# ilyakurdyukov/jpeg-quantsmooth

Hardware: AMD Instinct MI355X
Metric: 8x8 blocks/s at q=3 niter=3 (higher is better)
Workload: dtype f32

## Files before the change

### jpeg-quantsmooth_amd/csrc/qs_device.h

```cpp
#pragma once
#include <stdint.h>

#define QS_APRON_X 16
#define QS_LDS_PITCH 65
#define QS_TAB_MAX 272

enum {
  QS_DIAGONALS = 1, QS_JOINT_YUV = 2, QS_UPSAMPLE_UV = 4, QS_LOW_QUALITY = 8,
  QS_NO_REBALANCE = 16, QS_NO_REBALANCE_UV = 32, QS_TRANSCODE = 64
};

struct QsConsts {
  int32_t nat[64];
  int32_t q[64];
  int32_t qraw[64];
  int32_t x1[64];
  int32_t x2[64];
  float   range[64];
  int32_t qn[64], x1n[64], x2n[64];
  int32_t tab_size;
  int32_t pad[15];
  float   tab[64 * QS_TAB_MAX];
  int32_t rec[64][4];
};
enum {
  QS_REC_H_ANY = 1,
  QS_REC_H_SKIP4 = 2,
  QS_REC_H_EVEN = 4,
  QS_REC_V_ANY = 8,
  QS_REC_V_SKIP4 = 16,
  QS_REC_V_EVEN = 32,
  QS_REC_LDS_SHIFT = 6,
  QS_REC_NXT_SHIFT = 12,
  QS_REC_Q1 = 1 << 21
};

static inline int qs_plane_pitch(int wblk) {
  return ((wblk * 8 + QS_APRON_X + 1) + 63) & ~63;
}

#define QS_MAX_PLANES 56
struct QsPlaneRef {
  const QsConsts* cst;
  int16_t* coef;
  uint8_t* plane;
  int32_t* status;
  int32_t wblk, hblk, pitch;
  int32_t mode;
  uint8_t* plane_next;
};
enum {
  QS_PLANE_REBALANCE = 1,
  QS_PLANE_REP_TOP = 2,
  QS_PLANE_REP_BOT = 4
};
struct QsPlaneAux {
  const uint8_t* p[QS_MAX_PLANES];
};
struct QsPlaneSet {
  int32_t n, pad;
  int32_t wave0[QS_MAX_PLANES + 2];
  QsPlaneRef ref[QS_MAX_PLANES];
};
```

### jpeg-quantsmooth_amd/csrc/qs_kernels.hip

```cpp
#include <hip/hip_runtime.h>
#include <stdint.h>
#include <stdlib.h>
#include "qs_device.h"



__device__ __forceinline__ void wave_lds_sync() {
  __builtin_amdgcn_fence(__ATOMIC_RELEASE, "wavefront");
  __builtin_amdgcn_wave_barrier();
  __builtin_amdgcn_fence(__ATOMIC_ACQUIRE, "wavefront");
}

__device__ __forceinline__ uint32_t mulc(uint32_t a, int c) {
  return (uint32_t)__mul24((int)a, c);
}

__device__ __forceinline__ uint32_t lshl13_add(uint32_t x, uint32_t b) {
  uint32_t r;
  asm("v_lshl_add_u32 %0, %1, 13, %2" : "=v"(r) : "v"(x), "v"(b));
  return r;
}

__device__ __forceinline__ void idct8(uint32_t (&v)[8], uint32_t bias) {
  uint32_t z1, z2, z3, z4, z5, t0, t1, t2, t3, e0, e1, e2, e3;
// ... 176 lines not shown
               "ds_read_i16 %6, %16 offset:780\n\tds_read_i16 %7, %16 offset:782\n\t" \
               "ds_read_i16 %8, %16 offset:1040\n\tds_read_i16 %9, %16 offset:1042\n\t" \
               "ds_read_i16 %10, %16 offset:1300\n\tds_read_i16 %11, %16 offset:1302\n\t" \
               "ds_read_i16 %12, %16 offset:1560\n\tds_read_i16 %13, %16 offset:1562\n\t" \
               "ds_read_i16 %14, %16 offset:1820\n\tds_read_i16 %15, %16 offset:1822\n\t" \
               "s_waitcnt lgkmcnt(0)" \
               : "=&v"(W[(N0) + 0]), "=&v"(W[(N0) + 1]), "=&v"(W[(N0) + 2]), "=&v"(W[(N0) + 3]), \
                 "=&v"(W[(N0) + 4]), "=&v"(W[(N0) + 5]), "=&v"(W[(N0) + 6]), "=&v"(W[(N0) + 7]), \
                 "=&v"(W[(N0) + 8]), "=&v"(W[(N0) + 9]), "=&v"(W[(N0) + 10]), "=&v"(W[(N0) + 11]), \
                 "=&v"(W[(N0) + 12]), "=&v"(W[(N0) + 13]), "=&v"(W[(N0) + 14]), "=&v"(W[(N0) + 15]) \
               : "v"(BASE) : "memory")
__device__ __forceinline__ void lds_read_block_i16(const uint32_t* col, uint32_t (&ws)[64]) {
  typedef const __attribute__((address_space(3))) uint32_t* lds_ptr;
  const uint32_t a0 = (uint32_t)(uintptr_t)(lds_ptr)col;
  const uint32_t a1 = a0 + 8 * 260, a2 = a0 + 16 * 260, a3 = a0 + 24 * 260;
  QS_LDS16_GROUP(a0, ws, 0);
  QS_LDS16_GROUP(a1, ws, 16);
  QS_LDS16_GROUP(a2, ws, 32);
  QS_LDS16_GROUP(a3, ws, 48);
}

#define QS_PIX_SCALE 0.000244140625f
#define QS_TERM_D(D, W) { \
    float u_ = __builtin_amdgcn_fmed3f(Rs - __builtin_fabsf(D), 0.0f, 1.0f); \
    float t_ = u_ * u_; \
    float x_ = (D) * t_; \
    float y_ = (W) * t_; \
    num = num + x_ * y_; \
    den = den + y_ * y_; }
#define QS_TERM(A, B, W) { float d_ = (A) - (B); QS_TERM_D(d_, W) }

typedef float qs_w16 __attribute__((ext_vector_type(16)));
typedef int qs_i4 __attribute__((ext_vector_type(4)));
#define QS_SWAIT(BUF) asm volatile("s_waitcnt lgkmcnt(0)" : "+s"(BUF) : : "memory")

#define QS_WAVES_PER_WG 4
#define QS_SMOOTH_MIN_WAVES 3
#define QS_RESIDENT_WG (256 * QS_SMOOTH_MIN_WAVES * 4 / QS_WAVES_PER_WG)
#define QS_PRIO_SLOW 3
#define QS_PRIO_TERMS 0

#define QS_TERM_OPT(COND, A, B, W) { float d_, t_; \
        asm volatile( \
          "s_cmp_lg_u32 %[c], 0\n\t" \
          "s_cbranch_scc1 1f\n\t" \
          "v_sub_f32 %[d], %[a], %[b]\n\t" \
          "v_sub_f32 %[t], %[r], |%[d]| clamp\n\t" \
          "v_mul_f32 %[t], %[t], %[t]\n\t" \
          "v_mul_f32 %[d], %[d], %[t]\n\t" \
          "v_mul_f32 %[t], %[w], %[t]\n\t" \
          "v_mul_f32 %[d], %[d], %[t]\n\t" \
          "v_add_f32 %[n], %[n], %[d]\n\t" \
          "v_mul_f32 %[d], %[t], %[t]\n\t" \
          "v_add_f32 %[e], %[e], %[d]\n" \
          "1:" \
          : [n] "+v"(num), [e] "+v"(den), [d] "=&v"(d_), [t] "=&v"(t_) \
          : [a] "v"(A), [b] "v"(B), [w] "s"(W), [r] "s"(Rs), [c] "s"(COND) : "scc"); }
#define QS_TERM_ASM(A, B, W) { float d_, t_; \
        asm volatile( \
          "v_sub_f32 %[d], %[a], %[b]\n\t" \
          "v_sub_f32 %[t], %[r], |%[d]| clamp\n\t" \
          "v_mul_f32 %[t], %[t], %[t]\n\t" \
          "v_mul_f32 %[d], %[d], %[t]\n\t" \
          "v_mul_f32 %[t], %[w], %[t]\n\t" \
          "v_mul_f32 %[d], %[d], %[t]\n\t" \
          "v_add_f32 %[n], %[n], %[d]\n\t" \
          "v_mul_f32 %[d], %[t], %[t]\n\t" \
          "v_add_f32 %[e], %[e], %[d]" \
          : [n] "+v"(num), [e] "+v"(den), [d] "=&v"(d_), [t] "=&v"(t_) \
          : [a] "v"(A), [b] "v"(B), [w] "s"(W), [r] "s"(Rs)); }

#define QS_TERM_D_ASM(D, W) { float d_, t_; \
        asm volatile( \
          "v_sub_f32 %[t], %[r], |%[a]| clamp\n\t" \
          "v_mul_f32 %[t], %[t], %[t]\n\t" \
          "v_mul_f32 %[d], %[a], %[t]\n\t" \
          "v_mul_f32 %[t], %[w], %[t]\n\t" \
          "v_mul_f32 %[d], %[d], %[t]\n\t" \
          "v_add_f32 %[n], %[n], %[d]\n\t" \
          "v_mul_f32 %[d], %[t], %[t]\n\t" \
          "v_add_f32 %[e], %[e], %[d]" \
          : [n] "+v"(num), [e] "+v"(den), [d] "=&v"(d_), [t] "=&v"(t_) \
          : [a] "v"(D), [w] "s"(W), [r] "s"(Rs)); }
#define QS_HOIST 20
#ifndef QS_HOIST_DIAG
#define QS_HOIST_DIAG 32
#endif
#ifndef QS_Q1_SKIP
#define QS_Q1_SKIP 1
#endif
#ifndef QS_STASH
#define QS_STASH 1
#endif

#define QS_SMOOTH_KERNEL_NAME qs_smooth_plane_kernel
#include "qs_smooth_kernel.inc"
#undef QS_SMOOTH_KERNEL_NAME
#define QS_SMOOTH_KERNEL_NAME qs_smooth_set_kernel
#define QS_SMOOTH_SET 1
#include "qs_smooth_kernel.inc"
#undef QS_SMOOTH_KERNEL_NAME
#undef QS_SMOOTH_SET

#define QS_DP_KERNEL_NAME qs_smooth_dp_kernel
#include "qs_smooth_dp_kernel.inc"
#undef QS_DP_KERNEL_NAME
#define QS_DP_KERNEL_NAME qs_smooth_dp_set_kernel
#define QS_DP_SET 1
#include "qs_smooth_dp_kernel.inc"
#undef QS_DP_KERNEL_NAME
#undef QS_DP_SET

__global__ void __launch_bounds__(256)
qs_clamp_kernel(int16_t* __restrict__ coef, size_t nvec) {
  size_t i = (size_t)blockIdx.x * 256 + threadIdx.x;
  const size_t stride = (size_t)gridDim.x * 256;
  uint4* p = reinterpret_cast<uint4*>(coef);
  for (; i < nvec; i += stride) {
    uint4 v = p[i];
    uint32_t d[4] = {v.x, v.y, v.z, v.w};
#pragma unroll
    for (int c = 0; c < 4; ++c) {
      int lo = (int16_t)(d[c] & 0xffff), hi = (int32_t)d[c] >> 16;
      lo = min(max(lo, -1023), 1023); hi = min(max(hi, -1023), 1023);
      d[c] = ((uint32_t)lo & 0xffffu) | ((uint32_t)hi << 16);
    }
    p[i] = make_uint4(d[0], d[1], d[2], d[3]);
  }
}

__global__ void __launch_bounds__(256)
qs_dequant_kernel(const QsConsts* __restrict__ cst, int16_t* __restrict__ coef, size_t nvec) {
  size_t i = (size_t)blockIdx.x * 256 + threadIdx.x;
  const size_t stride = (size_t)gridDim.x * 256;
  uint4* p = reinterpret_cast<uint4*>(coef);
  for (; i < nvec; i += stride) {
    uint4 v = p[i];
    uint32_t d[4] = {v.x, v.y, v.z, v.w};
    const int j = (int)(i & 7);
#pragma unroll
    for (int c = 0; c < 4; ++c) {
      int lo = (int16_t)(d[c] & 0xffff), hi = (int32_t)d[c] >> 16;
      lo *= cst->qraw[j * 8 + c * 2]; hi *= cst->qraw[j * 8 + c * 2 + 1];
      d[c] = ((uint32_t)lo & 0xffffu) | ((uint32_t)hi << 16);
    }
    p[i] = make_uint4(d[0], d[1], d[2], d[3]);
  }
}

#include "qs_launch.h"

void qs_launch_idct_plane(const QsConsts* cst, int16_t* coef, uint8_t* plane, int wblk, int hblk,
                          int first, int rep_top, int rep_bot, int* status, hipStream_t s) {
  const int nblk = wblk * hblk;
  hipLaunchKernelGGL(qs_idct_plane_kernel, dim3((nblk + 255) / 256), dim3(256), 0, s,
                     cst, coef, plane, wblk, hblk, qs_plane_pitch(wblk), first, rep_top, rep_bot, status);
}

#define QS_DP_WAVES 4
static int qs_dp_waves(int groups) {
  static const int on = [] { const char* v = getenv("QS_HIP_DP"); return v ? atoi(v) : 1; }();
  static const int lim = [] { const char* v = getenv("QS_HIP_DP_GROUPS"); return v ? atoi(v) : 768; }();
  static const int lim2 = [] { const char* v = getenv("QS_HIP_DP_GROUPS2"); return v ? atoi(v) : 1536; }();
  if (!on) return 0;
  return groups <= lim ? QS_DP_WAVES : groups <= lim2 ? 2 : 0;
}

void qs_launch_smooth_plane(const QsConsts* cst, int16_t* coef, const uint8_t* plane, uint8_t* plane_next, int rep_top, int rep_bot,
                            int wblk, int hblk, int diag, int rebalance, int final_clamp, int blk_begin, int blk_end, hipStream_t s) {
// ... 53 lines not shown
```

### jpeg-quantsmooth_amd/csrc/qs_smooth_kernel.inc

```
template <bool DIAG>
__global__ void __launch_bounds__(64 * QS_WAVES_PER_WG, QS_SMOOTH_MIN_WAVES)
#ifdef QS_SMOOTH_SET
QS_SMOOTH_KERNEL_NAME(const QsPlaneSet set, int final_clamp) {
  __shared__ uint32_t lds_all[QS_WAVES_PER_WG][32 * QS_LDS_PITCH];
#if QS_STASH
  __shared__ uint32_t stash_all[QS_WAVES_PER_WG][2 * 8 * 64];
#endif
  const int lane = threadIdx.x & 63, wave = threadIdx.x >> 6;
  uint32_t* lds = lds_all[wave];
  uint32_t* col = lds + lane;
  const int gw = __builtin_amdgcn_readfirstlane((int)(blockIdx.x * QS_WAVES_PER_WG + wave));
  if (gw >= set.wave0[set.n]) return;
  const int pi = qs_set_find(set, gw);
  const QsConsts* __restrict__ cst = set.ref[pi].cst;
  int16_t* __restrict__ coef = set.ref[pi].coef;
  const uint8_t* __restrict__ plane = set.ref[pi].plane;
  const int wblk = set.ref[pi].wblk, hblk = set.ref[pi].hblk, pitch = set.ref[pi].pitch;
  const int rebalance = set.ref[pi].mode & QS_PLANE_REBALANCE;
  const int nblk = wblk * hblk;
  const int base = (gw - set.wave0[pi]) * 64;
  (void)hblk;
#else
QS_SMOOTH_KERNEL_NAME(const QsConsts* __restrict__ cst, int16_t* __restrict__ coef,
                       const uint8_t* __restrict__ plane, uint8_t* __restrict__ plane_next, int rep,
                       int wblk, int hblk, int pitch,
                       int rebalance, int final_clamp, int blk_begin, int blk_end) {
  __shared__ uint32_t lds_all[QS_WAVES_PER_WG][32 * QS_LDS_PITCH];
#if QS_STASH
  __shared__ uint32_t stash_all[QS_WAVES_PER_WG][2 * 8 * 64];
#endif
  const int lane = threadIdx.x & 63, wave = threadIdx.x >> 6;
  uint32_t* lds = lds_all[wave];
  uint32_t* col = lds + lane;
  const int nblk = blk_end;
  const int base = blk_begin + (blockIdx.x * QS_WAVES_PER_WG + wave) * 64;
#endif
  if (base >= nblk) return;
  const int tail_prio = __builtin_amdgcn_readfirstlane(
      (gridDim.x > QS_RESIDENT_WG && blockIdx.x >= (gridDim.x / QS_RESIDENT_WG) * QS_RESIDENT_WG) ? 1 : 0);
  const int nvec = min(64, nblk - base) * 8;
#ifdef QS_STAGGER
  { unsigned hwid; asm volatile("s_getreg_b32 %0, hwreg(HW_REG_HW_ID)" : "=s"(hwid)); if (hwid & 1u) __builtin_amdgcn_s_sleep(QS_STAGGER); }
#endif

  uint4* gsrc = reinterpret_cast<uint4*>(coef) + (size_t)base * 8;
  {
    const int m0 = (lane & 7) * 4;
#pragma unroll
    for (int j = 0; j < 8; ++j) {
      const int idx = j * 64 + lane;
      uint4 v = make_uint4(0, 0, 0, 0);
      if (idx < nvec) v = gsrc[idx];
      uint32_t* dst = lds + m0 * QS_LDS_PITCH + (j * 8 + (lane >> 3));
      dst[0] = v.x; dst[QS_LDS_PITCH] = v.y; dst[2 * QS_LDS_PITCH] = v.z; dst[3 * QS_LDS_PITCH] = v.w;
    }
  }

  const int blk = min(base + lane, nblk - 1);
  const int by = blk / wblk, bx = blk - by * wblk;
  const uint8_t* org = plane + (size_t)(by * 8 + 1) * pitch + QS_APRON_X + bx * 8;
  uint32_t edge[8];
  {
    const uint2 t = *reinterpret_cast<const uint2*>(org - pitch);
    const uint2 b = *reinterpret_cast<const uint2*>(org + (size_t)8 * pitch);
    edge[0] = t.x; edge[1] = t.y; edge[2] = b.x; edge[3] = b.y;
    uint32_t l[8], r[8];
#pragma unroll
    for (int y = 0; y < 8; ++y) {
      l[y] = org[(ptrdiff_t)y * pitch - 1];
      r[y] = org[(ptrdiff_t)y * pitch + 8];
    }
    edge[4] = l[0] | (l[1] << 8) | (l[2] << 16) | (l[3] << 24);
    edge[5] = l[4] | (l[5] << 8) | (l[6] << 16) | (l[7] << 24);
    edge[6] = r[0] | (r[1] << 8) | (r[2] << 16) | (r[3] << 24);
    edge[7] = r[4] | (r[5] << 8) | (r[6] << 16) | (r[7] << 24);
  }
  wave_lds_sync();

  constexpr int TS = DIAG ? 272 : 160;
  float px[64];
  float bd[32];
  constexpr int NH = DIAG ? QS_HOIST_DIAG : QS_HOIST;
  float hd[NH];

  int kfirst = 63;
#if QS_STASH
  int stash_hi = 0;
#endif
  uint32_t chg = 0;
  long long reb_m0 = 0, reb_m1 = 0;
  const float* tabp = cst->tab;
  const int32_t* recp = &cst->rec[0][0];
  qs_w16 WA, WB;
  qs_i4 REC;
  qs_i4 RECN;
  asm volatile("s_load_dwordx4 %0, %2, %3\n\ts_load_dwordx16 %1, %4, %5\n\ts_waitcnt lgkmcnt(0)"
               : "=&s"(REC), "=&s"(WA) : "s"(recp), "s"(63u * 16u), "s"(tabp), "s"((uint32_t)63 * (TS * 4)) : "memory");
  RECN = REC;

#pragma unroll 1
  for (int g = 0; g < 14; ++g) {
    __builtin_amdgcn_s_setprio(QS_PRIO_SLOW);
    if (g == 0 || __builtin_amdgcn_ballot_w64(chg != 0) != 0) {
      chg = 0;
      uint32_t ws[64];
      lds_read_block_i16(col, ws);
#if QS_STASH
      {
        uint32_t* stash = stash_all[wave] + lane;
#pragma unroll
        for (int x = 0; x < 8; ++x) {
          uint32_t c[8];
          const bool low = x <= 1, high = x >= 6;
          const int slot = (x == 0 || x == 7) ? 0 : 1;
          bool reuse = false, store = false;
          if (low) { reuse = g >= 1 && g <= 7 - x; store = g == 0; }
          if (high) {
            const int fin = 15 - x;
            const bool have = (stash_hi >> (x - 6)) & 1;
            reuse = g >= fin && have; store = g >= fin && !have;
          }
          if ((low || high) && reuse) {
#pragma unroll
            for (int j = 0; j < 8; ++j) c[j] = stash[(slot * 8 + j) * 64];
          } else {
#pragma unroll
            for (int j = 0; j < 8; ++j) c[j] = ws[j * 8 + x];
            idct8(c, 1024u);
#pragma unroll
            for (int j = 0; j < 8; ++j) c[j] = (uint32_t)((int32_t)c[j] >> 11);
            if ((low || high) && store) {
#pragma unroll
              for (int j = 0; j < 8; ++j) stash[(slot * 8 + j) * 64] = c[j];
              if (high) stash_hi |= 1 << (x - 6);
            }
          }
#pragma unroll
          for (int j = 0; j < 8; ++j) ws[j * 8 + x] = c[j];
        }
      }
#else
      idct_pass1(ws);
#endif
#pragma unroll
      for (int y = 0; y < 8; ++y) {
        uint32_t row[8]; float o[8];
#pragma unroll
        for (int j = 0; j < 8; ++j) row[j] = ws[y * 8 + j];
        idct_pass2_row_f(row, o);
#pragma unroll
        for (int j = 0; j < 8; ++j) px[y * 8 + j] = o[j];
      }
#pragma unroll
      for (int e = 0; e < 8; ++e) asm volatile("" : "+v"(edge[e]));
#pragma unroll
      for (int x = 0; x < 8; ++x) {
        bd[x]      = px[x]         - pix_from_byte(edge[0 + (x >> 2)], x & 3);
        bd[8 + x]  = px[56 + x]    - pix_from_byte(edge[2 + (x >> 2)], x & 3);
        bd[16 + x] = px[x * 8]     - pix_from_byte(edge[4 + (x >> 2)], x & 3);
        bd[24 + x] = px[x * 8 + 7] - pix_from_byte(edge[6 + (x >> 2)], x & 3);
      }
#pragma unroll
      for (int t = 0; t < NH; ++t) hd[t] = px[(t / 7) * 8 + t % 7] - px[(t / 7) * 8 + t % 7 + 1];
    }
    const int len = min(g + 1, 15 - g);
    const int klast = max(kfirst - len + 1, 1);
#pragma unroll 1
    for (int k = kfirst; k >= klast; --k) {
#pragma unroll
      for (int p = 0; p < 64; ++p) asm volatile("" : "+v"(px[p]));
      const int md = REC[3];
      const int x2k = (REC[0] >> 16) & 31, qk = REC[1] & 0xffff, x1k = REC[1] >> 16;
      const uint32_t lds_off = ((uint32_t)md >> QS_REC_LDS_SHIFT) & 0x3fffu;
      int rs_bits = REC[2];
      asm volatile("" : "+s"(rs_bits));
      const float Rs = __builtin_bit_cast(float, rs_bits);
      const uint32_t kb = (uint32_t)k * (TS * 4);
      const uint32_t kb_nxt = kb - (uint32_t)(TS * 4);
      const uint32_t kb_s = (uint32_t)__builtin_amdgcn_readfirstlane((int)kb);
      const uint32_t kb_nxt_s = (uint32_t)__builtin_amdgcn_readfirstlane((int)kb_nxt);
      const uint32_t next_first = kb_nxt + (((uint32_t)md >> QS_REC_NXT_SHIFT) & 0x100u);
      const uint32_t after_V = DIAG ? kb + 640u : next_first;
      const uint32_t after_B = (md & QS_REC_V_ANY) ? kb + 384u : after_V;
#if QS_Q1_SKIP
      if (__builtin_expect(md & QS_REC_Q1, 0)) {
        {
          const int c0 = *reinterpret_cast<lds_i16*>(reinterpret_cast<char*>(col) + lds_off);
          reb_m0 += (long long)(c0 * c0);
          reb_m1 += (long long)(c0 * c0);
        }
        asm volatile("s_load_dwordx16 %0, %2, %3\n\ts_load_dwordx4 %1, %4, %5\n\ts_waitcnt lgkmcnt(0)"
                     : "=&s"(WA), "=&s"(RECN)
                     : "s"(tabp), "s"((uint32_t)__builtin_amdgcn_readfirstlane((int)next_first)), "s"(recp),
                       "s"((uint32_t)(k - 1) * 16u) : "memory");
        REC = RECN;
      } else
#endif
      {
      float num = 0.0f, den = 0.0f;
      asm volatile("s_setprio %c1\n\ts_cmp_eq_u32 %0, 0\n\ts_cbranch_scc1 1f\n\ts_setprio %c2\n1:"
                   : : "s"(tail_prio), "i"(QS_PRIO_TERMS), "i"(QS_PRIO_TERMS + 1) : "scc");

#define QS_ROW_D(W, Y) { \
        _Pragma("unroll") for (int x = 0; x < 7; ++x) { \
          QS_TERM(px[(Y) * 8 + x], px[(Y) * 8 + x + 9], W[x]) \
          QS_TERM(px[(Y) * 8 + x + 1], px[(Y) * 8 + x + 8], W[8 + x]) } }
#define QS_EDGE16(W, J0) { \
        _Pragma("unroll") for (int j = 0; j < 16; ++j) QS_TERM_D(bd[(J0) + j], W[j]) }
#define QS_HOISTED_TERM(T, WT) else if ((T) < NH) QS_TERM_D_ASM(hd[(T) % NH], WT)
#define QS_ROWS_H_M(W, Y0, MODE) { \
        _Pragma("unroll") for (int yy = 0; yy < 2; ++yy) \
        _Pragma("unroll") for (int x = 0; x < 7; ++x) { \
          if (((MODE) == 2 && (x & 1)) || ((MODE) == 1 && x == 3)) {} \
          QS_HOISTED_TERM(((Y0) + yy) * 7 + x, W[yy * 8 + x]) \
          else QS_TERM_ASM(px[((Y0) + yy) * 8 + x], px[((Y0) + yy) * 8 + x + 1], W[yy * 8 + x]) } }
#define QS_ROWS_V_M(W, Y0, NY, MODE) { \
        _Pragma("unroll") for (int yy = 0; yy < (NY); ++yy) \
        _Pragma("unroll") for (int x = 0; x < 8; ++x) { \
          if (((MODE) == 2 && (((Y0) + yy) & 1)) || ((MODE) == 1 && (Y0) + yy == 3)) {} \
          else QS_TERM_ASM(px[((Y0) + yy) * 8 + x], px[((Y0) + yy) * 8 + x + 8], W[yy * 8 + x]) } }

      const uint32_t rec_next = (uint32_t)(k - 1) * 16u;
#define QS_ISSUE(NXT, BYTEOFF) \
      asm volatile("s_load_dwordx16 %0, %3, %4" : "=&s"(NXT), "+v"(num), "+v"(den) \
                   : "s"(tabp), "s"((uint32_t)__builtin_amdgcn_readfirstlane((int)(BYTEOFF))) : "memory")
#define QS_ISSUE_K(NXT, IMM) \
      asm volatile("s_load_dwordx16 %0, %3, %4 offset:%c5" : "=&s"(NXT), "+v"(num), "+v"(den) \
                   : "s"(tabp), "s"(kb_s), "i"(IMM) : "memory")
#define QS_LAND(NXT) asm volatile("s_waitcnt lgkmcnt(0)" : "+s"(NXT), "+v"(num), "+v"(den) : : "memory")
#define QS_ISSUE_R(NXT, BYTEOFF) \
      asm volatile("s_load_dwordx16 %0, %4, %5\n\ts_load_dwordx4 %1, %6, %7" : "=&s"(NXT), "=&s"(RECN), "+v"(num), "+v"(den) \
                   : "s"(tabp), "s"((uint32_t)__builtin_amdgcn_readfirstlane((int)(BYTEOFF))), "s"(recp), "s"(rec_next) : "memory")
#define QS_LAND_R(NXT) asm volatile("s_waitcnt lgkmcnt(0)" : "+s"(NXT), "+s"(RECN), "+v"(num), "+v"(den) : : "memory")
#define QS_T4(O) "s_load_dword %1, %4, %5 offset:" #O "\n\ts_load_dword %1, %4, %5 offset:" #O "+0x40\n\ts_load_dword %1, %4, %5 offset:" #O "+0x80\n\ts_load_dword %1, %4, %5 offset:" #O "+0xc0\n\t"
#define QS_ISSUE_T(NXT, IMM) \
      uint32_t touch; \
      if (DIAG) asm volatile("s_load_dwordx16 %0, %4, %6 offset:%c7\n\t" QS_T4(0x0) QS_T4(0x100) QS_T4(0x200) QS_T4(0x300) "s_load_dword %1, %4, %5 offset:0x400" \
                   : "=&s"(NXT), "=&s"(touch), "+v"(num), "+v"(den) \
                   : "s"(tabp), "s"(kb_nxt_s), "s"(kb_s), "i"(IMM) : "memory"); \
      else      asm volatile("s_load_dwordx16 %0, %4, %6 offset:%c7\n\t" QS_T4(0x0) QS_T4(0x100) "s_load_dword %1, %4, %5 offset:0x200\n\ts_load_dword %1, %4, %5 offset:0x240" \
                   : "=&s"(NXT), "=&s"(touch), "+v"(num), "+v"(den) \
                   : "s"(tabp), "s"(kb_nxt_s), "s"(kb_s), "i"(IMM) : "memory")
#define QS_LAND_T(NXT) asm volatile("s_waitcnt lgkmcnt(0)" : "+s"(NXT), "+s"(touch), "+v"(num), "+v"(den) : : "memory")
#define QS_H_SECTION(MODE) { \
        QS_ISSUE_K(WB, 64);  QS_ROWS_H_M(WA, 0, MODE) QS_LAND(WB); \
        QS_ISSUE_K(WA, 128); QS_ROWS_H_M(WB, 2, MODE) QS_LAND(WA); \
        QS_ISSUE_K(WB, 192); QS_ROWS_H_M(WA, 4, MODE) QS_LAND(WB); \
        QS_ISSUE_K(WA, 256); QS_ROWS_H_M(WB, 6, MODE) QS_LAND(WA); }
      if (md & QS_REC_H_ANY) {
        if (md & QS_REC_H_SKIP4) QS_H_SECTION(2)
        else if (md & QS_REC_H_EVEN) QS_H_SECTION(1)
        else QS_H_SECTION(0)
      }
      QS_ISSUE_T(WB, 320); QS_EDGE16(WA, 0) QS_LAND_T(WB);
      if (!DIAG && !(md & QS_REC_V_ANY)) { QS_ISSUE_R(WA, after_B); QS_EDGE16(WB, 16) QS_LAND_R(WA); }
      else                   { QS_ISSUE(WA, after_B);   QS_EDGE16(WB, 16) QS_LAND(WA); }
#define QS_V_SECTION(MODE) { \
        QS_ISSUE_K(WB, 448); QS_ROWS_V_M(WA, 0, 2, MODE) QS_LAND(WB); \
        QS_ISSUE_K(WA, 512); QS_ROWS_V_M(WB, 2, 2, MODE) QS_LAND(WA); \
        QS_ISSUE_K(WB, 576); QS_ROWS_V_M(WA, 4, 2, MODE) QS_LAND(WB); \
        if (!DIAG) { QS_ISSUE_R(WA, after_V); QS_ROWS_V_M(WB, 6, 1, MODE) QS_LAND_R(WA); } \
        else       { QS_ISSUE(WA, after_V);   QS_ROWS_V_M(WB, 6, 1, MODE) QS_LAND(WA); } }
      if (md & QS_REC_V_ANY) {
        if (md & QS_REC_V_SKIP4) QS_V_SECTION(2)
        else if (md & QS_REC_V_EVEN) QS_V_SECTION(1)
        else QS_V_SECTION(0)
      }
      if (DIAG) {
        QS_ISSUE_K(WB, 704);  QS_ROW_D(WA, 0) QS_LAND(WB);
        QS_ISSUE_K(WA, 768);  QS_ROW_D(WB, 1) QS_LAND(WA);
        QS_ISSUE_K(WB, 832);  QS_ROW_D(WA, 2) QS_LAND(WB);
        QS_ISSUE_K(WA, 896);  QS_ROW_D(WB, 3) QS_LAND(WA);
        QS_ISSUE_K(WB, 960);  QS_ROW_D(WA, 4) QS_LAND(WB);
        QS_ISSUE_K(WA, 1024); QS_ROW_D(WB, 5) QS_LAND(WA);
        QS_ISSUE_R(WB, next_first); QS_ROW_D(WA, 6) QS_LAND_R(WB);
        WA = WB;
      }
#undef QS_ROWS_H_M
#undef QS_HOISTED_TERM
#undef QS_ROWS_V_M
#undef QS_H_SECTION
#undef QS_V_SECTION
#undef QS_ISSUE
#undef QS_ISSUE_K
#undef QS_LAND
#undef QS_ISSUE_R
#undef QS_LAND_R
#undef QS_ISSUE_T
#undef QS_LAND_T
#undef QS_T4

      __builtin_amdgcn_s_setprio(QS_PRIO_SLOW);
      lds_i16* const cptr = reinterpret_cast<lds_i16*>(reinterpret_cast<char*>(col) + lds_off);
      const int c0 = *cptr;
      const int r = f2i_x86(round_half_away((num / den) * 4096.0f));
      {
        int orig, lo, hi;
        interval(c0, qk, x1k, x2k, orig, lo, hi);
        int v = (int)((uint32_t)c0 - (uint32_t)r);
        v = min(max(v, lo), hi);
        *cptr = (lds_i16)v;
        chg |= (uint32_t)(v ^ c0);
        if (rebalance) {
          reb_m0 += (long long)(v * orig);
          reb_m1 += (long long)(orig * orig);
        }
      }
      REC = RECN;
      }
    }
    kfirst = klast - 1;
  }
  QS_SWAIT(WA);

  if (rebalance) {
    const long long m0 = reb_m0, m1 = reb_m1;
    if (m1 > m0) {
      const int mul = (int)(((m1 << 13) + (m0 >> 1)) / m0);
#pragma unroll 9
      for (int n = 1; n < 64; ++n) {
        const int c = lds_coef(col, n);
        int orig, lo, hi;
        interval(c, cst->qn[n], cst->x1n[n], cst->x2n[n], orig, lo, hi);
        int v = (c * mul + 0x1000) >> 13;
        v = min(max(v, lo), hi);
        lds_set_coef(col, n, v);
      }
    }
  }
  wave_lds_sync();

  {
    int lane2 = lane;
    asm volatile("" : "+v"(lane2));
    const int lane = lane2;
    const int m0 = (lane & 7) * 4;
#pragma unroll
    for (int j = 0; j < 8; ++j) {
      const int idx = j * 64 + lane;
      const uint32_t* s = lds + m0 * QS_LDS_PITCH + (j * 8 + (lane >> 3));
      uint32_t d[4] = {s[0], s[QS_LDS_PITCH], s[2 * QS_LDS_PITCH], s[3 * QS_LDS_PITCH]};
      if (final_clamp) {
#pragma unroll
        for (int c = 0; c < 4; ++c) {
          int lo = (int16_t)(d[c] & 0xffff), hi = (int32_t)d[c] >> 16;
          lo = min(max(lo, -1023), 1023); hi = min(max(hi, -1023), 1023);
          d[c] = ((uint32_t)lo & 0xffffu) | ((uint32_t)hi << 16);
        }
      }
      if (idx < nvec) gsrc[idx] = make_uint4(d[0], d[1], d[2], d[3]);
    }
  }

#ifdef QS_SMOOTH_SET
  int pi2 = pi;
  asm volatile("" : "+s"(pi2));
  uint8_t* __restrict__ plane_next = set.ref[pi2].plane_next;
  const int rep = set.ref[pi2].mode, wblk2 = set.ref[pi2].wblk, hblk2 = set.ref[pi2].hblk, pitch2 = set.ref[pi2].pitch;
#else
  const int wblk2 = wblk, hblk2 = hblk, pitch2 = pitch;
#endif
  if (plane_next) {
    uint32_t ws[64];
    lds_read_block_i16(col, ws);
    if (base + lane < nblk)
      idct_ws_to_plane(ws, plane_next, wblk2, hblk2, pitch2, rep & QS_PLANE_REP_TOP, rep & QS_PLANE_REP_BOT, base + lane);
  }
}

#undef QS_ROW_D
#undef QS_EDGE16
```

### jpeg-quantsmooth_amd/csrc/qs_tables.cpp

```cpp
#include <stdarg.h>
#include <math.h>
#include <mutex>

#include "qs_xfer.h"

static thread_local char g_err[512] = "";

int qs_fail(int code, const char* fmt, ...) {
  va_list ap; va_start(ap, fmt);
  vsnprintf(g_err, sizeof(g_err), fmt, ap);
  va_end(ap);
  return code;
}


extern "C" const char* qs_hip_last_error(void) { return g_err; }

extern "C" int qs_hip_device_count(void) {
  int n = 0;
  if (hipGetDeviceCount(&n) != hipSuccess) { (void)hipGetLastError(); return 0; }
  return n;
}

extern "C" size_t qs_hip_consts_bytes(void) { return sizeof(QsConsts); }
extern "C" size_t qs_hip_plane_pitch(int wblk) { return (size_t)qs_plane_pitch(wblk); }
extern "C" size_t qs_hip_plane_bytes(int wblk, int hblk) {
  return (size_t)qs_plane_pitch(wblk) * ((size_t)hblk * 8 + 2) + 64;
}
extern "C" size_t qs_hip_plane_row_offset(int wblk, int y) {
  return (size_t)qs_plane_pitch(wblk) * (size_t)(y + 1);
}
extern "C" void qs_hip_free(void* p) { if (p && !qsx::pinned_return(p)) free(p); }


static const unsigned char kZigzag[64] = {
  0, 1, 8, 16, 9, 2, 3, 10, 17, 24, 32, 25, 18, 11, 4, 5,
  12, 19, 26, 33, 40, 48, 41, 34, 27, 20, 13, 6, 7, 14, 21, 28,
  35, 42, 49, 56, 57, 50, 43, 36, 29, 22, 15, 23, 30, 37, 44, 51,
  58, 59, 52, 45, 38, 31, 39, 46, 53, 60, 61, 54, 47, 55, 62, 63
};

static void idct8f(const float* in, int is, float* out, int os, bool scale) {
  float z1, z2, z3, z4, z5, t0, t1, t2, t3, t4, t5, t6, t7;
  z2 = in[2 * is]; z3 = in[6 * is];
  z1 = (z2 + z3) * 0.541196100f;
  t2 = z1 - z3 * 1.847759065f;
  t3 = z1 + z2 * 0.765366865f;
  z2 = in[0]; z3 = in[4 * is];
  t0 = z2 + z3; t1 = z2 - z3;
  t4 = t0 + t3; t7 = t0 - t3; t5 = t1 + t2; t6 = t1 - t2;
  t0 = in[7 * is]; t1 = in[5 * is]; t2 = in[3 * is]; t3 = in[is];
  z1 = t0 + t3; z2 = t1 + t2; z3 = t0 + t2; z4 = t1 + t3;
  z5 = (z3 + z4) * 1.175875602f;
  t0 = t0 * 0.298631336f; t1 = t1 * 2.053119869f;
  t2 = t2 * 3.072711026f; t3 = t3 * 1.501321110f;
  z1 = z1 * 0.899976223f; z2 = z2 * 2.562915447f;
  z3 = z3 * 1.961570560f; z4 = z4 * 0.390180644f;
  z3 = z3 - z5; t0 = t0 - (z1 + z3); t2 = t2 - (z2 + z3);
  z4 = z4 - z5; t1 = t1 - (z2 + z4); t3 = t3 - (z1 + z4);
  float r[8] = { t4 + t3, t5 + t2, t6 + t1, t7 + t0, t7 - t0, t6 - t1, t5 - t2, t4 - t3 };
  for (int j = 0; j < 8; ++j) out[j * os] = scale ? r[j] * 0.125f : r[j];
}

static void impulse_response(int i, float T[64]) {
  float in[64], ws[64];
  memset(in, 0, sizeof(in)); in[i] = 1.0f;
  for (int x = 0; x < 8; ++x) idct8f(in + x, 8, ws + x, 8, false);
  for (int y = 0; y < 8; ++y) idct8f(ws + y * 8, 1, T + y * 8, 1, true);
}

struct WeightTables {
  float tab[2][64 * QS_TAB_MAX];
  int status[2];
  char msg[2][160];
};

static void build_tables(WeightTables& W, int diag) {
  const int ts = diag ? 272 : 160;
  const float b = diag ? 4.0f : 2.0f;
  float* tab = W.tab[diag];
  memset(tab, 0, sizeof(W.tab[diag]));
  W.status[diag] = QS_HIP_OK;
  for (int k = 0; k < 64; ++k) {
    const int i = kZigzag[k];
    float T[64], *w = tab + (size_t)k * ts;
// ... 12 lines not shown
        const int p = y * 8 + x;
        w[160 + 16 * y + x] = x < 7 ? T[p] - T[p + 9] : 0.0f;
        w[168 + 16 * y + x] = x < 7 ? T[p + 1] - T[p + 8] : 0.0f;
      }
  }
  for (int k = 1; k < 64; ++k) {
    const int i = kZigzag[k], u = i & 7, v = i >> 3;
    const float* w = tab + (size_t)k * ts;
    for (int y = 0; y < 8; ++y) for (int x = 0; x < 7; ++x)
      if (u && ((x + 1) * u) % 8 == 0 && w[y * 8 + x] != 0.0f) {
        W.status[diag] = QS_HIP_EINVAL;
        snprintf(W.msg[diag], sizeof(W.msg[diag]), "weight table: expected exact zero at k=%d h(%d,%d)", k, y, x);
      }
    for (int y = 0; y < 7; ++y) for (int x = 0; x < 8; ++x)
      if (v && ((y + 1) * v) % 8 == 0 && w[96 + y * 8 + x] != 0.0f) {
        W.status[diag] = QS_HIP_EINVAL;
        snprintf(W.msg[diag], sizeof(W.msg[diag]), "weight table: expected exact zero at k=%d v(%d,%d)", k, y, x);
      }
  }
  for (size_t j = 0; j < (size_t)64 * ts; ++j) {
    const float a = tab[j] < 0 ? -tab[j] : tab[j];
    if (a != 0.0f && a < 2.3283064e-10f ) {
      W.status[diag] = QS_HIP_EINVAL;
      snprintf(W.msg[diag], sizeof(W.msg[diag]), "weight table entry %g too small for the scaled evaluation", (double)a);
    }
  }
}

static const WeightTables& weight_tables() {
  static WeightTables* W = [] {
    WeightTables* w = new WeightTables;
    build_tables(*w, 0);
    build_tables(*w, 1);
    return w;
  }();
  return *W;
}

extern "C" int qs_hip_consts_build(void* host_out, const uint16_t quant[64], int flags) {
  if (!host_out || !quant) return qs_fail(QS_HIP_EINVAL, "qs_hip_consts_build: null argument");
  QsConsts* c = static_cast<QsConsts*>(host_out);
  const int diag = (flags & QS_DIAGONALS) != 0;
  const int ts = diag ? 272 : 160;
  const WeightTables& W = weight_tables();
  if (W.status[diag] != QS_HIP_OK) return qs_fail(W.status[diag], "%s", W.msg[diag]);
  memset(c, 0, offsetof(QsConsts, tab));
  c->tab_size = ts;
  int qn[64], x1n[64], x2n[64];
  for (int i = 0; i < 64; ++i) {
    unsigned q = quant[i] ? quant[i] : 1u, n = 0, t = q;
    while (t > 1) { t >>= 1; ++n; }
    unsigned x1 = ((0x10000u << n) + q - 1) / q;
    if (n) x1 |= x1 >> 16;
    const int sh = 15 - (int)n;
    qn[i] = (int)q; x1n[i] = (int16_t)(uint16_t)x1; x2n[i] = sh;
    c->qraw[i] = quant[i];
    c->qn[i] = qn[i]; c->x1n[i] = x1n[i]; c->x2n[i] = x2n[i];
  }
  for (int k = 0; k < 64; ++k) {
    const int i = kZigzag[k];
    c->nat[k] = i; c->q[k] = qn[i]; c->x1[k] = x1n[i]; c->x2[k] = x2n[i];
    c->range[k] = (float)(qn[i] * 2) * 0.000244140625f;
  }
  for (int k = 0; k < 64; ++k) {
    const int kn = k > 1 ? k - 1 : 1;
    c->rec[k][0] = c->nat[k] | (c->nat[kn] << 8) | (c->x2[k] << 16);
    c->rec[k][1] = (int32_t)(((uint32_t)c->q[k] & 0xffffu) | ((uint32_t)c->x1[k] << 16));
    memcpy(&c->rec[k][2], &c->range[k], sizeof(float));
    {
      const int i = c->nat[k], u = i & 7, v = i >> 3, i_nxt = c->nat[kn];
      int m = 0;
      if (u) m |= QS_REC_H_ANY;
      if (u == 4) m |= QS_REC_H_SKIP4;
      if (!(u & 1)) m |= QS_REC_H_EVEN;
      if (v) m |= QS_REC_V_ANY;
      if (v == 4) m |= QS_REC_V_SKIP4;
      if (!(v & 1)) m |= QS_REC_V_EVEN;
      m |= ((i >> 1) * QS_LDS_PITCH * 4 + (i & 1) * 2) << QS_REC_LDS_SHIFT;
      if (!(i_nxt & 7)) m |= 0x100 << QS_REC_NXT_SHIFT;
      if (c->q[k] == 1) m |= QS_REC_Q1;
      c->rec[k][3] = m;
    }
  }
  memcpy(c->tab, W.tab[diag], sizeof(c->tab));
  return QS_HIP_OK;
}
```

Before: 271.9 million.

## Pair same-quantizer coefficients within a diagonal to share the difference evaluation

Reorders each zigzag diagonal so coefficients with equal quantizer values sit next to each other, and evaluates such pairs together. The pixel-difference and range-weight terms are computed once and accumulated into two numerator/denominator pairs using each coefficient's own weight table. A host-side walk table carries the new order and pair flags, and pairing is turned off when too little work would be shared. The diagonal hoist count also drops, which adds register pressure elsewhere. Each pair is now computed from the same block state instead of one coefficient after the other, which may change results slightly.

```diff
diff --git a/jpeg-quantsmooth_amd/csrc/qs_device.h b/jpeg-quantsmooth_amd/csrc/qs_device.h
--- a/jpeg-quantsmooth_amd/csrc/qs_device.h
+++ b/jpeg-quantsmooth_amd/csrc/qs_device.h
@@ -22,6 +22,7 @@
   int32_t pad[15];
   float   tab[64 * QS_TAB_MAX];
   int32_t rec[64][4];
+  int32_t walk[64][4];
 };
 enum {
   QS_REC_H_ANY = 1,
@@ -32,8 +33,16 @@
   QS_REC_V_EVEN = 32,
   QS_REC_LDS_SHIFT = 6,
   QS_REC_NXT_SHIFT = 12,
-  QS_REC_Q1 = 1 << 21
+  QS_REC_Q1 = 1 << 21,
+  QS_REC_PAIR = 1 << 22,
+  QS_REC_PAIR_UH = 1 << 23,
+  QS_REC_PAIR_SH = 1 << 24,
+  QS_REC_PAIR_SV = 1 << 25,
+  QS_REC_PAIR_UVL = 1 << 26,
+  QS_REC_PAIR_UVF = 1 << 27
 };
+
+#define QS_PAIR_MIN_SHARED 1200
 
 static inline int qs_plane_pitch(int wblk) {
   return ((wblk * 8 + QS_APRON_X + 1) + 63) & ~63;
diff --git a/jpeg-quantsmooth_amd/csrc/qs_kernels.hip b/jpeg-quantsmooth_amd/csrc/qs_kernels.hip
--- a/jpeg-quantsmooth_amd/csrc/qs_kernels.hip
+++ b/jpeg-quantsmooth_amd/csrc/qs_kernels.hip
@@ -282,9 +282,40 @@
           "v_add_f32 %[e], %[e], %[d]" \
           : [n] "+v"(num), [e] "+v"(den), [d] "=&v"(d_), [t] "=&v"(t_) \
           : [a] "v"(D), [w] "s"(W), [r] "s"(Rs)); }
+#define QS_TERM2_WEIGHT_HALF \
+          "v_mul_f32 %[y], %[w0], %[t]\n\t" \
+          "v_mul_f32 %[p], %[d], %[y]\n\t" \
+          "v_add_f32 %[n0], %[n0], %[p]\n\t" \
+          "v_mul_f32 %[p], %[y], %[y]\n\t" \
+          "v_add_f32 %[e0], %[e0], %[p]\n\t" \
+          "v_mul_f32 %[y], %[w1], %[t]\n\t" \
+          "v_mul_f32 %[p], %[d], %[y]\n\t" \
+          "v_add_f32 %[n1], %[n1], %[p]\n\t" \
+          "v_mul_f32 %[p], %[y], %[y]\n\t" \
+          "v_add_f32 %[e1], %[e1], %[p]"
+#define QS_TERM2_ASM(A, B, W0, W1) { float d_, t_, y_, p_; \
+        asm volatile( \
+          "v_sub_f32 %[d], %[a], %[b]\n\t" \
+          "v_sub_f32 %[t], %[r], |%[d]| clamp\n\t" \
+          "v_mul_f32 %[t], %[t], %[t]\n\t" \
+          "v_mul_f32 %[d], %[d], %[t]\n\t" \
+          QS_TERM2_WEIGHT_HALF \
+          : [n0] "+v"(num), [e0] "+v"(den), [n1] "+v"(num2), [e1] "+v"(den2), \
+            [d] "=&v"(d_), [t] "=&v"(t_), [y] "=&v"(y_), [p] "=&v"(p_) \
+          : [a] "v"(A), [b] "v"(B), [w0] "s"(W0), [w1] "s"(W1), [r] "s"(Rs)); }
+#define QS_TERM2_D_ASM(D, W0, W1) { float d_, t_, y_, p_; \
+        asm volatile( \
+          "v_sub_f32 %[t], %[r], |%[a]| clamp\n\t" \
+          "v_mul_f32 %[t], %[t], %[t]\n\t" \
+          "v_mul_f32 %[d], %[a], %[t]\n\t" \
+          QS_TERM2_WEIGHT_HALF \
+          : [n0] "+v"(num), [e0] "+v"(den), [n1] "+v"(num2), [e1] "+v"(den2), \
+            [d] "=&v"(d_), [t] "=&v"(t_), [y] "=&v"(y_), [p] "=&v"(p_) \
+          : [a] "v"(D), [w0] "s"(W0), [w1] "s"(W1), [r] "s"(Rs)); }
+typedef float qs_w8 __attribute__((ext_vector_type(8)));
 #define QS_HOIST 20
 #ifndef QS_HOIST_DIAG
-#define QS_HOIST_DIAG 32
+#define QS_HOIST_DIAG 24
 #endif
 #ifndef QS_Q1_SKIP
 #define QS_Q1_SKIP 1
diff --git a/jpeg-quantsmooth_amd/csrc/qs_smooth_kernel.inc b/jpeg-quantsmooth_amd/csrc/qs_smooth_kernel.inc
--- a/jpeg-quantsmooth_amd/csrc/qs_smooth_kernel.inc
+++ b/jpeg-quantsmooth_amd/csrc/qs_smooth_kernel.inc
@@ -90,7 +90,7 @@
   uint32_t chg = 0;
   long long reb_m0 = 0, reb_m1 = 0;
   const float* tabp = cst->tab;
-  const int32_t* recp = &cst->rec[0][0];
+  const int32_t* recp = &cst->walk[0][0];
   qs_w16 WA, WB;
   qs_i4 REC;
   qs_i4 RECN;
@@ -175,13 +175,27 @@
       int rs_bits = REC[2];
       asm volatile("" : "+s"(rs_bits));
       const float Rs = __builtin_bit_cast(float, rs_bits);
-      const uint32_t kb = (uint32_t)k * (TS * 4);
-      const uint32_t kb_nxt = kb - (uint32_t)(TS * 4);
+      const uint32_t kb = (uint32_t)(REC[0] & 0xff) * (TS * 4);
+      const uint32_t kb_nxt = (uint32_t)((REC[0] >> 8) & 0xff) * (TS * 4);
       const uint32_t kb_s = (uint32_t)__builtin_amdgcn_readfirstlane((int)kb);
       const uint32_t kb_nxt_s = (uint32_t)__builtin_amdgcn_readfirstlane((int)kb_nxt);
       const uint32_t next_first = kb_nxt + (((uint32_t)md >> QS_REC_NXT_SHIFT) & 0x100u);
       const uint32_t after_V = DIAG ? kb + 640u : next_first;
       const uint32_t after_B = (md & QS_REC_V_ANY) ? kb + 384u : after_V;
+#define QS_UPDATE(NUM, DEN, LDS_OFF) { \
+        lds_i16* const cptr = reinterpret_cast<lds_i16*>(reinterpret_cast<char*>(col) + (LDS_OFF)); \
+        const int c0 = *cptr; \
+        const int r = f2i_x86(round_half_away(((NUM) / (DEN)) * 4096.0f)); \
+        int orig, lo, hi; \
+        interval(c0, qk, x1k, x2k, orig, lo, hi); \
+        int v = (int)((uint32_t)c0 - (uint32_t)r);   \
+        v = min(max(v, lo), hi); \
+        *cptr = (lds_i16)v; \
+        chg |= (uint32_t)(v ^ c0); \
+        if (rebalance) {                             \
+          reb_m0 += (long long)(v * orig); \
+          reb_m1 += (long long)(orig * orig); \
+        } }
 #if QS_Q1_SKIP
       if (__builtin_expect(md & QS_REC_Q1, 0)) {
         {
@@ -196,6 +210,129 @@
         REC = RECN;
       } else
 #endif
+      if (md & QS_REC_PAIR) {
+      float num = 0.0f, den = 0.0f, num2 = 0.0f, den2 = 0.0f;
+      qs_w8 P0, P1, Q0, Q1;
+      qs_i4 REC2;
+      const uint32_t kb2_s = kb_nxt_s;
+      asm volatile("s_setprio %c1\n\ts_cmp_eq_u32 %0, 0\n\ts_cbranch_scc1 1f\n\ts_setprio %c2\n1:"
+                   : : "s"(tail_prio), "i"(QS_PRIO_TERMS), "i"(QS_PRIO_TERMS + 1) : "scc");
+#define QS2_SUMS "+v"(num), "+v"(den), "+v"(num2), "+v"(den2)
+#define QS2_LOAD(A, B, IMM) \
+      asm volatile("s_load_dwordx8 %0, %6, %7 offset:%c9\n\ts_load_dwordx8 %1, %6, %8 offset:%c9\n\ts_waitcnt lgkmcnt(0)" \
+                   : "=&s"(A), "=&s"(B), QS2_SUMS : "s"(tabp), "s"(kb_s), "s"(kb2_s), "i"(IMM) : "memory")
+#define QS2_ISSUE(A, B, IMM) \
+      asm volatile("s_load_dwordx8 %0, %6, %7 offset:%c9\n\ts_load_dwordx8 %1, %6, %8 offset:%c9" \
+                   : "=&s"(A), "=&s"(B), QS2_SUMS : "s"(tabp), "s"(kb_s), "s"(kb2_s), "i"(IMM) : "memory")
+#define QS2_LAND(A, B) asm volatile("s_waitcnt lgkmcnt(0)" : "+s"(A), "+s"(B), QS2_SUMS : : "memory")
+#define QS1_LOAD(A, ROW, IMM) \
+      asm volatile("s_load_dwordx8 %0, %5, %6 offset:%c7\n\ts_waitcnt lgkmcnt(0)" \
+                   : "=&s"(A), QS2_SUMS : "s"(tabp), "s"(ROW), "i"(IMM) : "memory")
+#define QS1_ISSUE(A, ROW, IMM) \
+      asm volatile("s_load_dwordx8 %0, %5, %6 offset:%c7" : "=&s"(A), QS2_SUMS : "s"(tabp), "s"(ROW), "i"(IMM) : "memory")
+#define QS1_LAND(A) asm volatile("s_waitcnt lgkmcnt(0)" : "+s"(A), QS2_SUMS : : "memory")
+#define QS_ROW_H2(W0, W1, Y) { \
+        _Pragma("unroll") for (int x = 0; x < 7; ++x) { \
+          if ((Y) * 7 + x < NH) QS_TERM2_D_ASM(hd[((Y) * 7 + x) % NH], W0[x], W1[x]) \
+          else QS_TERM2_ASM(px[(Y) * 8 + x], px[(Y) * 8 + x + 1], W0[x], W1[x]) } }
+#define QS_ROW_H1(W, Y) { \
+        _Pragma("unroll") for (int x = 0; x < 7; ++x) { \
+          if ((Y) * 7 + x < NH) QS_TERM_D_ASM(hd[((Y) * 7 + x) % NH], W[x]) \
+          else QS_TERM_ASM(px[(Y) * 8 + x], px[(Y) * 8 + x + 1], W[x]) } }
+#define QS_ROW_V2(W0, W1, Y) { \
+        _Pragma("unroll") for (int x = 0; x < 8; ++x) QS_TERM2_ASM(px[(Y) * 8 + x], px[(Y) * 8 + x + 8], W0[x], W1[x]) }
+#define QS_ROW_V1(W, Y) { \
+        _Pragma("unroll") for (int x = 0; x < 8; ++x) QS_TERM_ASM(px[(Y) * 8 + x], px[(Y) * 8 + x + 8], W[x]) }
+#define QS_EDGE8_2(W0, W1, J0) { \
+        _Pragma("unroll") for (int j = 0; j < 8; ++j) QS_TERM2_D_ASM(bd[(J0) + j], W0[j], W1[j]) }
+      if (md & QS_REC_PAIR_UH) {
+        QS1_LOAD(P0, kb_s, 0);
+        QS1_ISSUE(Q0, kb_s, 32);  QS_ROW_H1(P0, 0) QS1_LAND(Q0);
+        QS1_ISSUE(P0, kb_s, 64);  QS_ROW_H1(Q0, 1) QS1_LAND(P0);
+        QS1_ISSUE(Q0, kb_s, 96);  QS_ROW_H1(P0, 2) QS1_LAND(Q0);
+        QS1_ISSUE(P0, kb_s, 128); QS_ROW_H1(Q0, 3) QS1_LAND(P0);
+        QS1_ISSUE(Q0, kb_s, 160); QS_ROW_H1(P0, 4) QS1_LAND(Q0);
+        QS1_ISSUE(P0, kb_s, 192); QS_ROW_H1(Q0, 5) QS1_LAND(P0);
+        QS1_ISSUE(Q0, kb_s, 224); QS_ROW_H1(P0, 6) QS1_LAND(Q0);
+        QS_ROW_H1(Q0, 7)
+      }
+      if (md & QS_REC_PAIR_SH) {
+        QS2_LOAD(P0, P1, 0);
+        QS2_ISSUE(Q0, Q1, 32);  QS_ROW_H2(P0, P1, 0) QS2_LAND(Q0, Q1);
+        QS2_ISSUE(P0, P1, 64);  QS_ROW_H2(Q0, Q1, 1) QS2_LAND(P0, P1);
+        QS2_ISSUE(Q0, Q1, 96);  QS_ROW_H2(P0, P1, 2) QS2_LAND(Q0, Q1);
+        QS2_ISSUE(P0, P1, 128); QS_ROW_H2(Q0, Q1, 3) QS2_LAND(P0, P1);
+        QS2_ISSUE(Q0, Q1, 160); QS_ROW_H2(P0, P1, 4) QS2_LAND(Q0, Q1);
+        QS2_ISSUE(P0, P1, 192); QS_ROW_H2(Q0, Q1, 5) QS2_LAND(P0, P1);
+        QS2_ISSUE(Q0, Q1, 224); QS_ROW_H2(P0, P1, 6) QS2_LAND(Q0, Q1);
+        QS_ROW_H2(Q0, Q1, 7)
+      }
+      asm volatile("s_load_dwordx8 %0, %7, %8 offset:256\n\ts_load_dwordx8 %1, %7, %9 offset:256\n\ts_load_dwordx4 %2, %10, %11\n\ts_waitcnt lgkmcnt(0)"
+                   : "=&s"(P0), "=&s"(P1), "=&s"(REC2), QS2_SUMS
+                   : "s"(tabp), "s"(kb_s), "s"(kb2_s), "s"(recp), "s"((uint32_t)(k - 1) * 16u) : "memory");
+      QS2_ISSUE(Q0, Q1, 288); QS_EDGE8_2(P0, P1, 0)  QS2_LAND(Q0, Q1);
+      QS2_ISSUE(P0, P1, 320); QS_EDGE8_2(Q0, Q1, 8)  QS2_LAND(P0, P1);
+      QS2_ISSUE(Q0, Q1, 352); QS_EDGE8_2(P0, P1, 16) QS2_LAND(Q0, Q1);
+      QS_EDGE8_2(Q0, Q1, 24)
+      if (md & QS_REC_PAIR_SV) {
+        QS2_LOAD(P0, P1, 384);
+        QS2_ISSUE(Q0, Q1, 416); QS_ROW_V2(P0, P1, 0) QS2_LAND(Q0, Q1);
+        QS2_ISSUE(P0, P1, 448); QS_ROW_V2(Q0, Q1, 1) QS2_LAND(P0, P1);
+        QS2_ISSUE(Q0, Q1, 480); QS_ROW_V2(P0, P1, 2) QS2_LAND(Q0, Q1);
+        QS2_ISSUE(P0, P1, 512); QS_ROW_V2(Q0, Q1, 3) QS2_LAND(P0, P1);
+        QS2_ISSUE(Q0, Q1, 544); QS_ROW_V2(P0, P1, 4) QS2_LAND(Q0, Q1);
+        QS2_ISSUE(P0, P1, 576); QS_ROW_V2(Q0, Q1, 5) QS2_LAND(P0, P1);
+        QS_ROW_V2(P0, P1, 6)
+      }
+      if (md & (QS_REC_PAIR_UVL | QS_REC_PAIR_UVF)) {
+        const bool fol = (md & QS_REC_PAIR_UVF) != 0;
+        const uint32_t row_s = fol ? kb2_s : kb_s;
+        if (fol) { float t = num; num = num2; num2 = t; t = den; den = den2; den2 = t; }
+        QS1_LOAD(P0, row_s, 384);
+        QS1_ISSUE(Q0, row_s, 416); QS_ROW_V1(P0, 0) QS1_LAND(Q0);
+        QS1_ISSUE(P0, row_s, 448); QS_ROW_V1(Q0, 1) QS1_LAND(P0);
+        QS1_ISSUE(Q0, row_s, 480); QS_ROW_V1(P0, 2) QS1_LAND(Q0);
+        QS1_ISSUE(P0, row_s, 512); QS_ROW_V1(Q0, 3) QS1_LAND(P0);
+        QS1_ISSUE(Q0, row_s, 544); QS_ROW_V1(P0, 4) QS1_LAND(Q0);
+        QS1_ISSUE(P0, row_s, 576); QS_ROW_V1(Q0, 5) QS1_LAND(P0);
+        QS_ROW_V1(P0, 6)
+        if (fol) { float t = num; num = num2; num2 = t; t = den; den = den2; den2 = t; }
+      }
+      if (DIAG) {
+#define QS_ROW_D2(Y) { \
+        QS2_LOAD(P0, P1, 640 + (Y) * 64); QS2_LOAD(Q0, Q1, 672 + (Y) * 64); \
+        _Pragma("unroll") for (int x = 0; x < 7; ++x) { \
+          QS_TERM2_ASM(px[(Y) * 8 + x], px[(Y) * 8 + x + 9], P0[x], P1[x]) \
+          QS_TERM2_ASM(px[(Y) * 8 + x + 1], px[(Y) * 8 + x + 8], Q0[x], Q1[x]) } }
+        QS_ROW_D2(0) QS_ROW_D2(1) QS_ROW_D2(2) QS_ROW_D2(3) QS_ROW_D2(4) QS_ROW_D2(5) QS_ROW_D2(6)
+#undef QS_ROW_D2
+      }
+      {
+        const uint32_t first2 = (uint32_t)((REC2[0] >> 8) & 0xff) * (TS * 4) + (((uint32_t)REC2[3] >> QS_REC_NXT_SHIFT) & 0x100u);
+        asm volatile("s_load_dwordx16 %0, %2, %3\n\ts_load_dwordx4 %1, %4, %5\n\ts_waitcnt lgkmcnt(0)"
+                     : "=&s"(WA), "=&s"(RECN)
+                     : "s"(tabp), "s"((uint32_t)__builtin_amdgcn_readfirstlane((int)first2)), "s"(recp),
+                       "s"((uint32_t)(k - 2) * 16u) : "memory");
+      }
+      __builtin_amdgcn_s_setprio(QS_PRIO_SLOW);
+      const uint32_t lds_off2 = ((uint32_t)REC2[3] >> QS_REC_LDS_SHIFT) & 0x3fffu;
+      QS_UPDATE(num, den, lds_off)
+      QS_UPDATE(num2, den2, lds_off2)
+      REC = RECN;
+      --k;
+#undef QS2_SUMS
+#undef QS2_LOAD
+#undef QS2_ISSUE
+#undef QS2_LAND
+#undef QS1_LOAD
+#undef QS1_ISSUE
+#undef QS1_LAND
+#undef QS_ROW_H2
+#undef QS_ROW_H1
+#undef QS_ROW_V2
+#undef QS_ROW_V1
+#undef QS_EDGE8_2
+      } else
       {
       float num = 0.0f, den = 0.0f;
       asm volatile("s_setprio %c1\n\ts_cmp_eq_u32 %0, 0\n\ts_cbranch_scc1 1f\n\ts_setprio %c2\n1:"
@@ -291,23 +428,10 @@
 #undef QS_T4
 
       __builtin_amdgcn_s_setprio(QS_PRIO_SLOW);
-      lds_i16* const cptr = reinterpret_cast<lds_i16*>(reinterpret_cast<char*>(col) + lds_off);
-      const int c0 = *cptr;
-      const int r = f2i_x86(round_half_away((num / den) * 4096.0f));
-      {
-        int orig, lo, hi;
-        interval(c0, qk, x1k, x2k, orig, lo, hi);
-        int v = (int)((uint32_t)c0 - (uint32_t)r);
-        v = min(max(v, lo), hi);
-        *cptr = (lds_i16)v;
-        chg |= (uint32_t)(v ^ c0);
-        if (rebalance) {
-          reb_m0 += (long long)(v * orig);
-          reb_m1 += (long long)(orig * orig);
-        }
-      }
+      QS_UPDATE(num, den, lds_off)
       REC = RECN;
       }
+#undef QS_UPDATE
     }
     kfirst = klast - 1;
   }
diff --git a/jpeg-quantsmooth_amd/csrc/qs_tables.cpp b/jpeg-quantsmooth_amd/csrc/qs_tables.cpp
--- a/jpeg-quantsmooth_amd/csrc/qs_tables.cpp
+++ b/jpeg-quantsmooth_amd/csrc/qs_tables.cpp
@@ -1,6 +1,7 @@
 #include <stdarg.h>
 #include <math.h>
 #include <mutex>
+#include <stdlib.h>
 
 #include "qs_xfer.h"
 
@@ -179,6 +180,51 @@
       c->rec[k][3] = m;
     }
   }
+  {
+    int order[64], lead[64], grp[64];
+    for (int k = 0; k < 64; ++k) { order[k] = k; lead[k] = 0; grp[k] = 0; }
+    for (int s = 1, hi = 1; s <= 14; ++s) {
+      const int len = s < 8 ? s + 1 : 15 - s;
+      bool used[8] = {false};
+      int pos = hi + len - 1;
+      for (int a = len - 1; a >= 0; --a) {
+        if (used[a]) continue;
+        const int za = hi + a;
+        int mem[8], n = 0;
+        for (int b = a; b >= 0; --b)
+          if (!used[b] && c->q[hi + b] == c->q[za] && c->q[za] > 1) mem[n++] = hi + b;
+        if (n < 2) { used[a] = true; order[pos--] = za; continue; }
+        for (int m = 0; m < n; ++m) { used[mem[m] - hi] = true; grp[mem[m]] = mem[n - 1]; }
+        for (int m = 0; m + 1 < n; m += 2) {
+          int L = mem[m], F = mem[m + 1];
+          if (!(c->nat[L] & 7)) { const int t = L; L = F; F = t; }
+          const int hL = (c->nat[L] & 7) != 0, hF = (c->nat[F] & 7) != 0, vL = (c->nat[L] >> 3) != 0, vF = (c->nat[F] >> 3) != 0;
+          lead[pos] = QS_REC_PAIR | (hL && hF ? QS_REC_PAIR_SH : hL ? QS_REC_PAIR_UH : 0) |
+                      (vL && vF ? QS_REC_PAIR_SV : vL ? QS_REC_PAIR_UVL : vF ? QS_REC_PAIR_UVF : 0);
+          order[pos--] = L; order[pos--] = F;
+        }
+        if (n & 1) order[pos--] = mem[n - 1];
+      }
+      hi += len;
+    }
+    {
+      static const int min_shared = [] { const char* v = getenv("QS_HIP_PAIR_MIN"); return v ? atoi(v) : QS_PAIR_MIN_SHARED; }();
+      int shared = 0;
+      for (int p = 0; p < 64; ++p)
+        if (lead[p]) shared += 32 + (diag ? 98 : 0) + ((lead[p] & QS_REC_PAIR_SH) ? 56 : 0) + ((lead[p] & QS_REC_PAIR_SV) ? 56 : 0);
+      if (shared < min_shared)
+        for (int p = 0; p < 64; ++p) { order[p] = p; lead[p] = 0; }
+    }
+    for (int p = 0; p < 64; ++p) {
+      const int z = order[p], zn = order[p > 1 ? p - 1 : 1];
+      c->walk[p][0] = z | (zn << 8) | (c->x2[z] << 16) | (grp[z] << 24);
+      c->walk[p][1] = c->rec[z][1];
+      c->walk[p][2] = c->rec[z][2];
+      int m = c->rec[z][3] & ~(0x100 << QS_REC_NXT_SHIFT);
+      if (!(c->nat[zn] & 7)) m |= 0x100 << QS_REC_NXT_SHIFT;
+      c->walk[p][3] = m | lead[p];
+    }
+  }
   memcpy(c->tab, W.tab[diag], sizeof(c->tab));
   return QS_HIP_OK;
 }
```

Result: slower. 266.2 million (-2.1%).
